# apple/swift-homomorphic-encryption

Measured on NVIDIA B200. Metric: BFV ct*ct mults/sec at N=8192, 4 coefficient moduli, higher is better.
Workload: dtype u64

## Files before the change

swift-homomorphic-encryption_b200/csrc/context.cu:

```cuda
#include "context.hpp"

#include <cuda_runtime.h>

#include <cmath>
#include <cstdlib>
#include <cstring>

#include "hostmath.hpp"
#include "ntt_fast.cuh"

namespace hecuda {
using namespace host;


static void fill_barrett(u64 p, u64 &mu1, u64 &mu_hi, u64 &mu_lo) {
    mu1 = (u64)(((u128)1 << 64) / p);
    u128 mu = (p & (p - 1)) == 0 ? ((u128)1 << (128 - (bit_length(p) - 1))) : (~(u128)0) / p;
    mu_hi = (u64)(mu >> 64);
    mu_lo = (u64)mu;
}

static bool build_slot(HostSlot &hs, u64 p, int64_t n, int logn, u64 t, std::vector<ulonglong2> &tw,
                       std::vector<ulonglong2> &itw, std::string &err) {
    if (!is_prime(p) || (p - 1) % (2 * (u64)n) != 0) {
        err = "invalidNttModulus: " + std::to_string(p) + " is not a prime = 1 mod 2N";
        return false;
    }
    if (p >= (1ull << 62)) {
        err = "invalidModulus: " + std::to_string(p) + " exceeds 2^62 - 1";
        return false;
    }
    ModSlot &d = hs.dev;
    std::memset(&d, 0, sizeof(d));
    d.p = p;
    fill_barrett(p, d.mu1, d.mu_hi, d.mu_lo);
    d.bits = bit_length(p);
    d.s_prod = d.bits - 2;
    d.mu_prod = (u64)(((u128)1 << (d.bits + 62)) / p);
    d.red_shift = d.bits > 12 ? d.bits - 12 : 0;
    d.red_recip = (u32)((((u128)1) << (d.red_shift + 32)) / p);
    const u64 psi = min_primitive_root(2 * (u64)n, p);
    const u64 psi_inv = invmod(psi, p);
    hs.roots.assign(n, 1);
    hs.inv_roots.assign(n, 1);
    u64 pw = 1, ipw = 1;
    for (int64_t i = 0; i < n; ++i) {
        unsigned r = bitrev((unsigned)i, logn);
        hs.roots[r] = pw;
        hs.inv_roots[r] = ipw;
        pw = mulmod(pw, psi, p);
        ipw = mulmod(ipw, psi_inv, p);
    }
    tw.resize(n);
    itw.resize(n);
    for (int64_t i = 0; i < n; ++i) {
        tw[i] = make_ulonglong2(hs.roots[i], shoup_factor(hs.roots[i], p));
        itw[i] = make_ulonglong2(hs.inv_roots[i], shoup_factor(hs.inv_roots[i], p));
    }
    const u64 n_inv = invmod((u64)n % p, p);
    const u64 w1_inv = n > 1 ? hs.inv_roots[1] : 1;
    d.r64 = (u64)(((u128)1 << 64) % p);
    {
        u64 inv = p;
        for (int i = 0; i < 6; ++i) inv *= 2 - p * inv;
        d.ninv = 0 - inv;
    }
    const u64 scalings[3] = {1 % p, mulmod(t % p, d.r64, p), d.r64};
    for (int k = 0; k < 3; ++k) {
        ModSlot::InvScale &sc = d.inv_scale[k];
        sc.c0 = mulmod(n_inv, scalings[k], p);
        sc.c0p = shoup_factor(sc.c0, p);
        sc.c1 = mulmod(sc.c0, w1_inv, p);
        sc.c1p = shoup_factor(sc.c1, p);
    }
    return true;
}

static DivRoundConsts build_divround(const std::vector<u64> &base) {
    DivRoundConsts c;
    std::memset(&c, 0, sizeof(c));
    c.l = (int)base.size();
    c.last = base.back();
    c.half = c.last >> 1;
    for (int i = 0; i + 1 < c.l; ++i) {
        const u64 m = base[i];
        c.m[i] = m;
        c.mu1[i] = (u64)(((u128)1 << 64) / m);
        c.half_mod[i] = c.half % m;
        c.inv_w[i] = invmod(c.last % m, m);
        c.inv_wp[i] = shoup_factor(c.inv_w[i], m);
    }
    return c;
}

Context *Context::create(int64_t n, const u64 *coeff_moduli, int nmod, u64 t, std::string &err, int word_bits) {
    if (word_bits != 64 && word_bits != 32) { err = "invalidEncryptionParameters: word size must be 32 or 64"; return nullptr; }
    for (int i = 0; i < nmod; ++i)
        if (coeff_moduli[i] >> (word_bits - 2)) { err = "invalidModulus: " + std::to_string(coeff_moduli[i]) + " exceeds the maximum of this word size"; return nullptr; }
    if (n < 2 || (n & (n - 1)) || n > (1 << 17)) { err = "invalidDegree: N must be a power of two in [2, 2^17]"; return nullptr; }
    if (n > (1 << fast::kSplitLogN)) { err = "unsupportedHeOperation: polynomial degrees above 2^" + std::to_string(fast::kSplitLogN) + " are not supported by the NTT kernels"; return nullptr; }
    if (nmod < 1) { err = "invalidEncryptionParameters: need at least one coefficient modulus"; return nullptr; }
    if (nmod > kMaxL) { err = "invalidEncryptionParameters: more than " + std::to_string(kMaxL) + " coefficient moduli (EncryptionParameters.swift:148)"; return nullptr; }
    if (t < 2) { err = "invalidEncryptionParameters: plaintext modulus"; return nullptr; }
    for (int i = 0; i < nmod; ++i)
        for (int j = 0; j < i; ++j)
            if (coeff_moduli[i] == coeff_moduli[j]) { err = "coprimeModuli: repeated coefficient modulus"; return nullptr; }

    Context *c = new Context();
    c->n = n;
    c->logn = bit_length((u64)n) - 1;
    c->has_ks = nmod >= 2;
    c->L = c->has_ks ? nmod - 1 : 1;
    c->t = t;
    c->word_bits = word_bits;
    c->mtilde = word_bits == 64 ? (1ull << 32) : (1ull << 16);
    c->gamma = word_bits == 64 ? ((1ull << 62) - 40797) : ((1ull << 30) - 20405);
    const u64 kMTilde = c->mtilde;
    cudaGetDevice(&c->device);
    c->sm_count = 1;
    cudaDeviceGetAttribute(&c->sm_count, cudaDevAttrMultiProcessorCount, c->device);
    const int L = c->L;
    c->q.assign(coeff_moduli, coeff_moduli + L);
    c->q_ks = c->has_ks ? coeff_moduli[L] : 0;
    for (u64 qi : c->q)
        if (t >= qi) { err = "invalidEncryptionParameters: plaintext modulus must be below every coefficient modulus"; delete c; return nullptr; }
    c->bsk = smallest_ntt_primes(word_bits - 3, L + 1, (u64)n);
    if ((int)c->bsk.size() != L + 1) { err = "notEnoughPrimes for Bsk"; delete c; return nullptr; }
    for (u64 b : c->bsk)
        for (int i = 0; i < nmod; ++i)
            if (b == coeff_moduli[i]) { err = "coprimeModuli: coefficient modulus collides with the BEHZ base"; delete c; return nullptr; }

    c->aux = c->bsk;
    {
        const char *env = std::getenv("HECUDA_AUX_BASE");
        const bool want_fast = !(env && std::string(env) == "reference");
        const int widths[2] = {30, 55};
        double log_q = 0;
        for (u64 v : c->q) log_q += std::log2((double)v);
        const double log_n = (double)c->logn, log_t = std::log2((double)t);
        for (int wi = 0; wi < 2 && want_fast && c->aux == c->bsk && word_bits == 64; ++wi) {
            const bool h_primes = fast::kNarrowHEnabled && std::getenv("HECUDA_AUX_H_PRIMES") != nullptr;
            std::vector<u64> cand = (widths[wi] == 55 && h_primes) ? smallest_ntt_primes(55, L + 1 + nmod, 1ull << 31)
                                                                   : smallest_ntt_primes(widths[wi], L + 1 + nmod, (u64)n);
            std::vector<u64> pick;
            for (u64 v : cand) {
                bool used = false;
                for (int i = 0; i < nmod; ++i) used |= coeff_moduli[i] == v;
                if (!used && (int)pick.size() < L + 1) pick.push_back(v);
            }
            double log_aux = 0, log_aux_l = 0;
            for (size_t j = 0; j < pick.size(); ++j) {
                log_aux += std::log2((double)pick[j]);
                if ((int)j < L) log_aux_l += std::log2((double)pick[j]);
            }
            const bool enough = (int)pick.size() == L + 1 && log_aux >= log_q + log_n + 4 &&
                                log_aux_l + std::log2((double)pick.back()) >= log_t + log_n + log_q + 5;
            if (enough) c->aux = pick;
        }
    }
    c->aux_is_reference = c->aux == c->bsk;

    const int nslots = c->aux_is_reference ? 2 * L + 2 : 3 * L + 3;
    c->slots.resize(nslots);
    std::vector<u64> slot_mod(nslots);
    for (int i = 0; i < L; ++i) slot_mod[c->slot_q(i)] = c->q[i];
    for (int j = 0; j <= L; ++j) slot_mod[c->slot_bsk(j)] = c->bsk[j];
    slot_mod[c->slot_ks()] = c->q_ks;
    if (!c->aux_is_reference)
        for (int j = 0; j <= L; ++j) slot_mod[c->slot_aux(j)] = c->aux[j];
    const size_t table_bytes = sizeof(ulonglong2) * (size_t)n;
    const bool fast = c->logn >= fast::kMinLogN && c->logn <= fast::kMaxLogN;
    const bool split = c->logn == fast::kSplitLogN;
    const int half_logn = c->logn - 1;
    const int64_t half_n = n / 2;
    const int threads = (int)((split ? half_n : n) / 16);
    const size_t tr_bytes = (fast || split) ? sizeof(ulonglong2) * (size_t)15 * threads : 0;
    const size_t half_bytes = sizeof(ulonglong2) * (size_t)half_n;
    const size_t slot_bytes = 2 * table_bytes + (split ? 2 * (2 * half_bytes + 2 * tr_bytes) : 2 * tr_bytes);
    if (cudaMalloc(&c->d_pool, slot_bytes * nslots) != cudaSuccess) { err = "cudaMalloc failed for twiddle tables"; delete c; return nullptr; }
    std::vector<ulonglong2> tw, itw, tr(15 * (size_t)threads), itr(15 * (size_t)threads), twh, itwh;
    std::vector<ModSlot> dev_slots(split ? 3 * nslots : nslots);
    c->split_slot_base = split ? nslots : 0;
    for (int s = 0; s < nslots; ++s) {
        if (s == c->slot_ks() && !c->has_ks) {
            std::memset(&c->slots[s].dev, 0, sizeof(ModSlot));
            dev_slots[s] = c->slots[s].dev;
            continue;
        }
        if (!build_slot(c->slots[s], slot_mod[s], n, c->logn, t, tw, itw, err)) { delete c; return nullptr; }
        char *base = (char *)c->d_pool + slot_bytes * s;
        cudaMemcpy(base, tw.data(), table_bytes, cudaMemcpyHostToDevice);
        cudaMemcpy(base + table_bytes, itw.data(), table_bytes, cudaMemcpyHostToDevice);
        c->slots[s].dev.tw = (const ulonglong2 *)base;
        c->slots[s].dev.itw = (const ulonglong2 *)(base + table_bytes);
        if (fast) {
            for (int k = 0; k < 15; ++k)
                for (int tau = 0; tau < threads; ++tau) {
                    tr[(size_t)k * threads + tau] = tw[fast::fwd_last_source(c->logn, k, tau)];
                    itr[(size_t)k * threads + tau] = itw[fast::inv_first_source(c->logn, k, tau)];
                }
            cudaMemcpy(base + 2 * table_bytes, tr.data(), tr_bytes, cudaMemcpyHostToDevice);
            cudaMemcpy(base + 2 * table_bytes + tr_bytes, itr.data(), tr_bytes, cudaMemcpyHostToDevice);
            c->slots[s].dev.tw_t = (const ulonglong2 *)(base + 2 * table_bytes);
            c->slots[s].dev.itw_t = (const ulonglong2 *)(base + 2 * table_bytes + tr_bytes);
        }
        dev_slots[s] = c->slots[s].dev;
        if (split) {
            for (int hh = 0; hh < 2; ++hh) {
                twh.assign(half_n, tw[0]);
                itwh.assign(half_n, itw[0]);
                for (int64_t i = 1; i < half_n; ++i) {
                    const int sp = bit_length((u64)i) - 1;
                    const int64_t src = ((int64_t)(2 + hh) << sp) + (i - ((int64_t)1 << sp));
                    twh[i] = tw[src];
                    itwh[i] = itw[src];
                }
                for (int k = 0; k < 15; ++k)
                    for (int tau = 0; tau < threads; ++tau) {
                        tr[(size_t)k * threads + tau] = twh[fast::fwd_last_source(half_logn, k, tau)];
                        itr[(size_t)k * threads + tau] = itwh[fast::inv_first_source(half_logn, k, tau)];
                    }
                char *hb = base + 2 * table_bytes + hh * (2 * half_bytes + 2 * tr_bytes);
// ... 203 lines not shown
```

swift-homomorphic-encryption_b200/csrc/context.hpp:

```cpp
#pragma once
#include <cstdint>
#include <string>
#include <vector>

#include "modarith.cuh"

namespace hecuda {

constexpr int kMaxL = 32;
constexpr int kMaxSlots = 3 * kMaxL + 3;
constexpr int kMaxRows = 2 * kMaxL + 1;

struct ModSlot {
    u64 p;
    u64 mu1;
    u64 mu_hi, mu_lo;
    u64 mu_prod;
    int s_prod;
    int bits;
    int red_shift;
    u32 red_recip;
    u64 ninv;
    u64 r64;
    struct InvScale { u64 c0, c0p, c1, c1p; } inv_scale[3];
    const ulonglong2 *tw;
    const ulonglong2 *itw;
    const ulonglong2 *tw_t;
    const ulonglong2 *itw_t;
};

enum { kScalePlain = 0, kScaleTMont = 1, kScaleMont = 2 };

struct NttRowMap {
    int rows_per_poly;
    int group;
    unsigned char slot[kMaxRows + 1];
    int src_mod;
    long long src_poly_stride;
    unsigned char src_slot[kMaxRows + 1];
};

struct LiftConsts {
    int L;
    int wide_sums;
    u64 b_mu1[kMaxL + 1];
    u64 q[kMaxL];
    u64 in_w[kMaxL], in_wp[kMaxL];
    u32 punct_mt[kMaxL];
    u32 neg_inv_q_mt;
    u32 mt_mask, mt_half;
    u64 neg_off[kMaxL + 1];
    u64 b[kMaxL + 1], b_ninv[kMaxL + 1];
    u64 mat[kMaxL + 1][kMaxL];
    u64 qr[kMaxL + 1];
};

// ... 75 lines not shown
```

swift-homomorphic-encryption_b200/csrc/hostmath.hpp:

```cpp
#pragma once
#include <cstdint>
#include <vector>

namespace hecuda {
namespace host {

typedef unsigned long long u64;
typedef unsigned __int128 u128;

inline u64 mulmod(u64 a, u64 b, u64 p) { return (u64)((u128)a * b % p); }

inline u64 powmod(u64 b, u64 e, u64 p) {
    u64 r = 1 % p;
    b %= p;
    for (; e; e >>= 1) {
        if (e & 1) r = mulmod(r, b, p);
        b = mulmod(b, b, p);
    }
    return r;
}

inline u64 invmod(u64 a, u64 m) {
    if (m == 0) return 0;
    a %= m;
// ... 11 lines not shown

inline bool is_prime(u64 n) {
    static const u64 witnesses[12] = {2, 3, 5, 7, 11, 13, 17, 19, 23, 29, 31, 37};
    if (n < 2) return false;
    for (u64 w : witnesses) {
        if (n == w) return true;
        if (n % w == 0) return false;
    }
    u64 d = n - 1;
    int r = 0;
    while (!(d & 1)) { d >>= 1; ++r; }
    for (u64 w : witnesses) {
        u64 x = powmod(w, d, n);
        if (x == 1 || x == n - 1) continue;
        bool composite = true;
        for (int i = 1; i < r && composite; ++i) {
            x = mulmod(x, x, n);
            if (x == n - 1) composite = false;
        }
        if (composite) return false;
    }
    return true;
}

inline std::vector<u64> smallest_ntt_primes(int bits, int count, u64 degree) {
    std::vector<u64> out;
    const u64 step = 2 * degree;
    const u64 lo = 1ull << (bits - 1), hi = (bits == 64) ? ~0ull : (1ull << bits);
    for (u64 c = lo + 1; c < hi && (int)out.size() < count; c += step)
        if (c % step == 1 && is_prime(c)) out.push_back(c);
    return out;
}

inline u64 min_primitive_root(u64 order, u64 p) {
    if (order < 2 || (order & (order - 1)) || (p - 1) % order) return 0;
    u64 gen = 0;
    for (u64 g = 2; g < p; ++g) {
        u64 r = powmod(g, (p - 1) / order, p);
        if (powmod(r, order / 2, p) == p - 1) { gen = r; break; }
    }
    if (!gen) return 0;
    u64 best = gen, cur = gen, g2 = mulmod(gen, gen, p);
    for (u64 k = 1; k < order; k += 2) {
        if (cur < best) best = cur;
        cur = mulmod(cur, g2, p);
    }
    return best;
}

inline unsigned bitrev(unsigned x, int bits) {
    unsigned r = 0;
    for (int i = 0; i < bits; ++i) r |= ((x >> i) & 1u) << (bits - 1 - i);
    return r;
}

inline int bit_length(u64 x) { return x ? 64 - __builtin_clzll(x) : 0; }

inline u64 prod_mod(const u64 *m, int n, u64 p) {
    u64 r = 1 % p;
    for (int i = 0; i < n; ++i) r = mulmod(r, m[i] % p, p);
    return r;
}
inline u64 punctured_mod(const u64 *m, int n, int skip, u64 p) {
    u64 r = 1 % p;
    for (int i = 0; i < n; ++i)
        if (i != skip) r = mulmod(r, m[i] % p, p);
// ... 7 lines not shown
```

swift-homomorphic-encryption_b200/csrc/ntt_fast.cu:

```cuda
#include <cuda.h>

#include <mutex>

#include <algorithm>
#include <cstdlib>
#include "kernels.cuh"
#include "ntt_fast.cuh"

namespace hecuda {
using namespace fast;

constexpr int kMaxRowList = 2 * (kMaxL + 1) * kMaxL;
struct RowList {
    int rows_per_poly;
    int count;
    unsigned short row[kMaxRowList];
    unsigned short slot[kMaxRowList];
    unsigned char flags[kMaxRowList];
    unsigned short src_row[kMaxRowList];
    long long src_poly_stride;
};

__device__ __forceinline__ u32 smem_u32(const void *p) { return (u32)__cvta_generic_to_shared(p); }
__device__ __forceinline__ void mbar_init(u64 *bar, int count) {
// ... 11 lines not shown
        "@!done bra WAIT_%=;\n\t}" ::"r"(smem_u32(bar)),
        "r"(parity)
        : "memory");
}
__device__ __forceinline__ void tma_load_1d(void *smem_dst, const void *gmem_src, u32 bytes, u64 *bar) {
    asm volatile("cp.async.bulk.shared::cluster.global.mbarrier::complete_tx::bytes [%0], [%1], %2, [%3];" ::"r"(smem_u32(smem_dst)),
                 "l"(gmem_src), "r"(bytes), "r"(smem_u32(bar))
                 : "memory");
}
__device__ __forceinline__ void tma_load_box(void *smem_dst, const CUtensorMap *map, int line, u64 *bar) {
    asm volatile("cp.async.bulk.tensor.2d.shared::cluster.global.tile.mbarrier::complete_tx::bytes [%0], [%1, {%2, %3}], [%4];" ::"r"(
                     smem_u32(smem_dst)),
                 "l"(map), "r"(0), "r"(line), "r"(smem_u32(bar))
                 : "memory");
}
__device__ __forceinline__ void tma_store_box(const CUtensorMap *map, int line, const void *smem_src) {
    asm volatile("cp.async.bulk.tensor.2d.global.shared::cta.tile.bulk_group [%0, {%1, %2}], [%3];" ::"l"(map), "r"(0), "r"(line),
                 "r"(smem_u32(smem_src))
                 : "memory");
}
__device__ __forceinline__ void tma_prefetch_box(const CUtensorMap *map, int line) {
    asm volatile("cp.async.bulk.prefetch.tensor.2d.L2.global.tile [%0, {%1, %2}];" ::"l"(map), "r"(0), "r"(line) : "memory");
}
__device__ __forceinline__ void tma_commit() { asm volatile("cp.async.bulk.commit_group;" ::: "memory"); }
__device__ __forceinline__ void tma_store_wait_read() { asm volatile("cp.async.bulk.wait_group.read 0;" ::: "memory"); }
__device__ __forceinline__ void tma_store_wait_all() { asm volatile("cp.async.bulk.wait_group 0;" ::: "memory"); }
__device__ __forceinline__ void fence_proxy_async_smem() { asm volatile("fence.proxy.async.shared::cta;" ::: "memory"); }

template <int LOGN, int CLS, int K>
__device__ __forceinline__ void fwd_row_pass(u64 (&x)[16], u64 *sm, int tau, const RowMod &m, bool reduce_in) {
    constexpr int P = plan_passes(LOGN), C = fwd_c(LOGN, K), LB = fwd_lb(LOGN, K);
    load_smem<LOGN, LB, C>(x, sm, tau);
    if (K == 0 && reduce_in) {
#pragma unroll
        for (int r = 0; r < 16; ++r) x[r] = barrett64(x[r], 0 - m.np, m.slot->mu1);
    }
    fwd_pass<LOGN, LB, C, CLS>(x, tau, m);
    if (K == P - 1) fwd_finish<CLS>(x, m);
    store_smem<LOGN, LB, C>(x, sm, tau);
}
template <int LOGN, int CLS>
__device__ __forceinline__ void fwd_row(u64 *sm, int tau, const RowMod &m, bool reduce_in) {
    constexpr int P = plan_passes(LOGN);
    u64 x[16];
    fwd_row_pass<LOGN, CLS, 0>(x, sm, tau, m, reduce_in);
    __syncthreads();
    fwd_row_pass<LOGN, CLS, 1>(x, sm, tau, m, false);
    __syncthreads();
    if (P == 4) {
        fwd_row_pass<LOGN, CLS, (P == 4 ? 2 : 1)>(x, sm, tau, m, false);
        __syncthreads();
    }
    fwd_row_pass<LOGN, CLS, P - 1>(x, sm, tau, m, false);
}

template <int LOGN, int CLS, int K>
__device__ __forceinline__ void inv_row_pass(u64 (&x)[16], u64 *sm, int tau, const RowMod &m) {
    constexpr int C = inv_c(LOGN, K), LB = inv_lb(LOGN, K);
    load_smem<LOGN, LB, C>(x, sm, tau);
    if (narrow_like(CLS) && K > 0 && inv_reduce_at(LOGN, K)) inv_reduce(x, m);
    inv_pass<LOGN, LB, C, CLS, inv_bound_in(LOGN, K)>(x, tau, m);
    if (K == plan_passes(LOGN) - 1 && m.partial) {
        if (CLS == kSmall) {
#pragma unroll
            for (int r = 0; r < 16; ++r) x[r] = csub32((u32)x[r], (u32)(0 - m.np));
        } else {
            reduce_small16(x, m);
        }
    }
    store_smem<LOGN, LB, C>(x, sm, tau);
}
template <int LOGN, int CLS>
__device__ __forceinline__ void inv_row(u64 *sm, int tau, const RowMod &m) {
    constexpr int P = plan_passes(LOGN);
    u64 x[16];
    inv_row_pass<LOGN, CLS, 0>(x, sm, tau, m);
    __syncthreads();
    inv_row_pass<LOGN, CLS, 1>(x, sm, tau, m);
    __syncthreads();
    if (P == 4) {
        inv_row_pass<LOGN, CLS, (P == 4 ? 2 : 1)>(x, sm, tau, m);
        __syncthreads();
    }
    inv_row_pass<LOGN, CLS, P - 1>(x, sm, tau, m);
}

template <int LOGN>
constexpr size_t ntt_smem_bytes() {
    return sizeof(u64) * ((size_t)1 << LOGN) + sizeof(ulonglong2) * ((size_t)1 << (LOGN - 4)) + 16;
}

template <int LOGN, bool INVERSE>
__global__ void __launch_bounds__((1 << LOGN) / 16, (1024 / ((1 << LOGN) / 16)))
    ntt_rows_kernel(const __grid_constant__ CUtensorMap map_in, const __grid_constant__ CUtensorMap map_out,
                    const ModSlot *__restrict__ slots, const __grid_constant__ RowList rl, const int polys,
                    const int scale_mode, const int debug_flags) {
    extern __shared__ __align__(1024) u64 sm[];
    constexpr int kLines = (1 << LOGN) / kLineWords;
    constexpr int kBoxes = kLines > kBoxLines ? kLines / kBoxLines : 1;
    constexpr int kLinesPerBox = kLines / kBoxes;
    constexpr u32 kRowBytes = (u32)sizeof(u64) << LOGN, kTwBytes = (u32)sizeof(ulonglong2) << (LOGN - 4);
    ulonglong2 *tw_cache = reinterpret_cast<ulonglong2 *>(sm + (1 << LOGN));
    u64 *bar_row = reinterpret_cast<u64 *>(tw_cache + (1 << (LOGN - 4)));
    u64 *bar_tw = bar_row + 1;
    const int tau = threadIdx.x;
    const int tasks = polys * rl.count;
    if (tau == 0) {
        if (smem_u32(sm) & 1023) __trap();
        mbar_init(bar_row, 1);
        mbar_init(bar_tw, 1);
    }
    __syncthreads();
    u32 phase_row = 0, phase_tw = 0;
    int cached_slot = -1;
    for (int task = blockIdx.x; task < tasks; task += gridDim.x) {
        const int which = task / polys;
        const int poly = task - which * polys;
        const int flags = rl.flags[which];
        const int slot = rl.slot[which];
        const ModSlot &S = slots[slot];
        const int64_t out_word = ((int64_t)poly * rl.rows_per_poly + rl.row[which]) << LOGN;
        const int64_t in_word = INVERSE ? out_word : (int64_t)poly * rl.src_poly_stride + ((int64_t)rl.src_row[which] << LOGN);
        const bool new_slot = slot != cached_slot;
        cached_slot = slot;
        if (tau == 0) {
            if (new_slot) {
                mbar_arrive_expect_tx(bar_tw, kTwBytes);
                tma_load_1d(tw_cache, INVERSE ? S.itw : S.tw, kTwBytes, bar_tw);
            }
            mbar_arrive_expect_tx(bar_row, kRowBytes);
            const int line = (int)(in_word >> 4);
#pragma unroll
            for (int b = 0; b < kBoxes; ++b) tma_load_box(sm + b * kLinesPerBox * kLineWords, &map_in, line + b * kLinesPerBox, bar_row);
            const int next = task + gridDim.x;
            if (next < tasks && !(debug_flags & 1)) {
                const int nw = next / polys;
                const int np_ = next - nw * polys;
                const int64_t nword = INVERSE ? ((int64_t)np_ * rl.rows_per_poly + rl.row[nw]) << LOGN
                                              : (int64_t)np_ * rl.src_poly_stride + ((int64_t)rl.src_row[nw] << LOGN);
#pragma unroll
                for (int b = 0; b < kBoxes; ++b) tma_prefetch_box(&map_in, (int)(nword >> 4) + b * kLinesPerBox);
            }
        }
        const int cls = flags & 7;
        RowMod m;
        m.np = 0 - S.p;
        m.kp = (cls == kWide || cls == kSmall) ? 2 * S.p : 4 * S.p;
        m.tw = nullptr;
        m.tw_s = smem_u32(tw_cache);
        m.slot = &S;
        m.scale_mode = INVERSE ? scale_mode : -1;
        m.partial = INVERSE && (flags & 16) != 0;
        if (new_slot) {
            mbar_wait(bar_tw, phase_tw);
            phase_tw ^= 1;
        }
        mbar_wait(bar_row, phase_row);
        phase_row ^= 1;
        if (debug_flags & 4) {
        } else
#ifndef HE_EXPERIMENT_ONLY_CLASS
        if (INVERSE) {
            if (kNarrowHEnabled && cls == kNarrowH) inv_row<LOGN, kNarrowHEnabled ? kNarrowH : kNarrow>(sm, tau, m);
            else if (cls == kNarrow) inv_row<LOGN, kNarrow>(sm, tau, m);
            else if (cls == kSmall) inv_row<LOGN, kSmall>(sm, tau, m);
            else if (cls == kMid) inv_row<LOGN, kMid>(sm, tau, m);
            else inv_row<LOGN, kWide>(sm, tau, m);
        } else {
            const bool reduce_in = (flags & 8) != 0;
            if (kNarrowHEnabled && cls == kNarrowH) fwd_row<LOGN, kNarrowHEnabled ? kNarrowH : kNarrow>(sm, tau, m, reduce_in);
            else if (cls == kNarrow) fwd_row<LOGN, kNarrow>(sm, tau, m, reduce_in);
            else if (cls == kSmall) fwd_row<LOGN, kSmall>(sm, tau, m, reduce_in);
            else if (cls == kMid) fwd_row<LOGN, kMid>(sm, tau, m, reduce_in);
            else fwd_row<LOGN, kWide>(sm, tau, m, reduce_in);
        }
#else
        if (INVERSE) inv_row<LOGN, HE_EXPERIMENT_ONLY_CLASS>(sm, tau, m);
        else fwd_row<LOGN, HE_EXPERIMENT_ONLY_CLASS>(sm, tau, m, (flags & 8) != 0);
#endif
        fence_proxy_async_smem();
        __syncthreads();
        if (tau == 0 && !(debug_flags & 2)) {
            const int line = (int)(out_word >> 4);
#pragma unroll
            for (int b = 0; b < kBoxes; ++b) tma_store_box(&map_out, line + b * kLinesPerBox, sm + b * kLinesPerBox * kLineWords);
            tma_commit();
            tma_store_wait_read();
        }
    }
    if (tau == 0) tma_store_wait_all();
}

static void build_row_list(const Context &ctx, const NttRowMap &map, bool inverse, RowList &rl) {
    rl.rows_per_poly = map.rows_per_poly;
    rl.count = 0;
    rl.src_poly_stride = map.src_mod ? map.src_poly_stride : (long long)map.rows_per_poly * ctx.n;
    static const int order[5] = {kWide, kMid, kNarrow, kNarrowH, kSmall};
    for (int oi = 0; oi < 5; ++oi) {
        const int cls = order[oi];
        for (int r = 0; r < map.rows_per_poly; ++r) {
            const int slot = map.slot[r / map.group];
            if (class_of_modulus(ctx.slots[slot].dev.p, ctx.slots[slot].dev.bits) != cls) continue;
            const int i = rl.count++;
            rl.row[i] = (unsigned short)r;
            rl.slot[i] = (unsigned short)slot;
            rl.src_row[i] = (unsigned short)(map.src_mod && !inverse ? r % map.src_mod : r);
            int flags = cls;
            if (map.src_mod && !inverse) {
                const u64 p = ctx.slots[slot].dev.p, src_p = ctx.slots[map.src_slot[r % map.src_mod]].dev.p;
                const u64 room = narrow_like(cls) ? 2u : cls == kMid ? 8u : cls == kSmall ? 1u : 4u;
                if (src_p > p && (src_p - 1) / p >= room) flags |= 8;
            }
            rl.flags[i] = (unsigned char)flags;
        }
    }
}

typedef CUresult (*EncodeTiledFn)(CUtensorMap *, CUtensorMapDataType, cuuint32_t, void *, const cuuint64_t *, const cuuint64_t *,
                                  const cuuint32_t *, const cuuint32_t *, CUtensorMapInterleave, CUtensorMapSwizzle,
                                  CUtensorMapL2promotion, CUtensorMapFloatOOBfill);
static EncodeTiledFn encode_tiled() {
    static EncodeTiledFn fn = [] {
        void *p = nullptr;
        cudaDriverEntryPointQueryResult q;
        if (cudaGetDriverEntryPoint("cuTensorMapEncodeTiled", &p, cudaEnableDefault, &q) != cudaSuccess || q != cudaDriverEntryPointSuccess)
            p = nullptr;
        return (EncodeTiledFn)p;
    }();
    return fn;
}
static bool make_line_map(CUtensorMap *map, const u64 *base, int logn) {
    EncodeTiledFn enc = encode_tiled();
    if (!enc || (reinterpret_cast<uintptr_t>(base) & 15)) return false;
    const int lines = (1 << logn) / kLineWords;
    const cuuint64_t dims[2] = {kLineWords, (cuuint64_t)1 << 31};
    const cuuint64_t strides[1] = {kLineWords * sizeof(u64)};
    const cuuint32_t box[2] = {kLineWords, (cuuint32_t)(lines > kBoxLines ? kBoxLines : lines)};
    const cuuint32_t elem_strides[2] = {1, 1};
    return enc(map, CU_TENSOR_MAP_DATA_TYPE_UINT64, 2, const_cast<u64 *>(base), dims, strides, box, elem_strides,
               CU_TENSOR_MAP_INTERLEAVE_NONE, CU_TENSOR_MAP_SWIZZLE_128B, CU_TENSOR_MAP_L2_PROMOTION_L2_128B,
               CU_TENSOR_MAP_FLOAT_OOB_FILL_NONE) == CUDA_SUCCESS;
}

template <int LOGN, bool INVERSE>
static cudaError_t launch_logn(const Context &ctx, const NttRowMap &map, const u64 *in, u64 *out, int64_t rows,
                               int scale_mode, cudaStream_t stream) {
    if (rows % map.rows_per_poly) return cudaErrorInvalidValue;
    if (rows == 0) return cudaSuccess;
    if (rows > 0x7fffffffLL) return cudaErrorInvalidValue;
    RowList rl;
    build_row_list(ctx, map, INVERSE, rl);
    if (rl.src_poly_stride % kLineWords) return cudaErrorInvalidValue;
    CUtensorMap map_in, map_out;
    if (!make_line_map(&map_in, in, LOGN) || !make_line_map(&map_out, out, LOGN)) return cudaErrorInvalidValue;
    const int polys = (int)(rows / map.rows_per_poly);
    constexpr int threads = (1 << LOGN) / 16;
    constexpr size_t smem = ntt_smem_bytes<LOGN>();
    auto k = ntt_rows_kernel<LOGN, INVERSE>;
    static int ctas_per_sm[64] = {0};
    static std::mutex mu;
    int per_sm;
    {
        std::lock_guard<std::mutex> lock(mu);
        int &c = ctas_per_sm[ctx.device & 63];
        if (c == 0) {
            cudaError_t e;
            if ((e = cudaFuncSetAttribute(k, cudaFuncAttributeMaxDynamicSharedMemorySize, (int)smem)) != cudaSuccess) return e;
            int n = 0;
            if ((e = cudaOccupancyMaxActiveBlocksPerMultiprocessor(&n, k, threads, smem)) != cudaSuccess) return e;
            if (n < 1) return cudaErrorInvalidConfiguration;
            c = n;
        }
        per_sm = c;
    }
    const int64_t grid = std::min<int64_t>(rows, (int64_t)ctx.sm_count * per_sm);
    ++g_kernel_launches;
    static const int debug_flags = [] {
        const char *env = std::getenv("HECUDA_NTT_DEBUG");
        return env ? std::atoi(env) : 0;
    }();
    k<<<(unsigned)grid, threads, smem, stream>>>(map_in, map_out, ctx.d_slots, rl, polys, scale_mode, debug_flags);
    return cudaGetLastError();
}

struct SplitRows {
    int rows_per_poly, count;
    unsigned short row[kMaxRowList];
    unsigned short src_row[kMaxRowList], slot[kMaxRowList];
    unsigned char reduce_in[kMaxRowList];
    long long src_poly_stride;
};
__global__ void __launch_bounds__(256) ntt_split_forward_kernel(const u64 *__restrict__ in, u64 *__restrict__ out,
                                                               const ModSlot *__restrict__ slots,
                                                               const __grid_constant__ SplitRows sr, int polys, int logn) {
    const int64_t n = (int64_t)1 << logn, half = n >> 1;
    const int which = blockIdx.y;
    const int64_t poly = blockIdx.z;
// ... 46 lines not shown
    sr.rows_per_poly = full.rows_per_poly;
    sr.count = full.count;
    sr.src_poly_stride = full.src_poly_stride;
    RowList rl;
    rl.rows_per_poly = 2 * full.rows_per_poly;
    rl.count = 2 * full.count;
    rl.src_poly_stride = (long long)rl.rows_per_poly << LOGN;
    for (int i = 0; i < full.count; ++i) {
        sr.row[i] = full.row[i];
        sr.slot[i] = full.slot[i];
        sr.src_row[i] = full.src_row[i];
        sr.reduce_in[i] = (unsigned char)((map.src_mod && !INVERSE) ? 1 : 0);
        for (int hh = 0; hh < 2; ++hh) {
            const int j = 2 * i + hh;
            rl.row[j] = (unsigned short)(2 * full.row[i] + hh);
            rl.src_row[j] = rl.row[j];
            rl.slot[j] = (unsigned short)(ctx.split_slot_base + 2 * full.slot[i] + hh);
            rl.flags[j] = (unsigned char)((full.flags[i] & 7) | (INVERSE ? 16 : 0));
        }
    }
    const dim3 egrid((unsigned)((ctx.n / 4 + 255) / 256), (unsigned)full.count, (unsigned)polys);
    if (!INVERSE) {
        ++g_kernel_launches;
        ntt_split_forward_kernel<<<egrid, 256, 0, stream>>>(in, out, ctx.d_slots, sr, polys, ctx.logn);
        cudaError_t e = cudaGetLastError();
        if (e != cudaSuccess) return e;
        in = out;
    }
    CUtensorMap map_in, map_out;
    if (!make_line_map(&map_in, in, LOGN) || !make_line_map(&map_out, out, LOGN)) return cudaErrorInvalidValue;
    {
        constexpr int threads = (1 << LOGN) / 16;
        constexpr size_t smem = ntt_smem_bytes<LOGN>();
        auto k = ntt_rows_kernel<LOGN, INVERSE>;
        cudaError_t e;
        if ((e = cudaFuncSetAttribute(k, cudaFuncAttributeMaxDynamicSharedMemorySize, (int)smem)) != cudaSuccess) return e;
        int per_sm = 0;
        if ((e = cudaOccupancyMaxActiveBlocksPerMultiprocessor(&per_sm, k, threads, smem)) != cudaSuccess) return e;
        if (per_sm < 1) return cudaErrorInvalidConfiguration;
        const int64_t grid = std::min<int64_t>(2 * rows, (int64_t)ctx.sm_count * per_sm);
        ++g_kernel_launches;
        k<<<(unsigned)grid, threads, smem, stream>>>(map_in, map_out, ctx.d_slots, rl, polys, scale_mode, 0);
        if ((e = cudaGetLastError()) != cudaSuccess) return e;
    }
    if (INVERSE) {
        ++g_kernel_launches;
        ntt_merge_inverse_kernel<<<egrid, 256, 0, stream>>>(out, ctx.d_slots, sr, polys, ctx.logn, scale_mode);
        return cudaGetLastError();
    }
    return cudaSuccess;
}

bool ntt_fast_supported(const Context &ctx) { return ctx.logn >= kMinLogN && ctx.logn <= kSplitLogN; }

template <bool INVERSE>
static cudaError_t launch_fast(const Context &ctx, const NttRowMap &map, const u64 *in, u64 *out, int64_t rows,
                               int scale_mode, cudaStream_t stream) {
    switch (ctx.logn) {
        case 10: return launch_logn<10, INVERSE>(ctx, map, in, out, rows, scale_mode, stream);
        case 11: return launch_logn<11, INVERSE>(ctx, map, in, out, rows, scale_mode, stream);
        case 12: return launch_logn<12, INVERSE>(ctx, map, in, out, rows, scale_mode, stream);
        case 13: return launch_logn<13, INVERSE>(ctx, map, in, out, rows, scale_mode, stream);
        case 14: return launch_logn<14, INVERSE>(ctx, map, in, out, rows, scale_mode, stream);
        case 15: return launch_split<INVERSE>(ctx, map, in, out, rows, scale_mode, stream);
        default: return cudaErrorInvalidValue;
    }
}
// ... 12 lines not shown
```

swift-homomorphic-encryption_b200/csrc/ntt_fast.cuh:

```cuda
#pragma once
#include "context.hpp"
#include "modarith.cuh"

namespace hecuda {
namespace fast {

constexpr int kMinLogN = 10, kMaxLogN = 14;
constexpr int kSplitLogN = 15;
constexpr int kNarrowBits = 55;
constexpr int kMidBits = 61;
constexpr int kSmallBits = 30;
enum { kNarrow = 0, kMid = 1, kWide = 2, kSmall = 3, kNarrowH = 4 };
HE_HD constexpr int class_of_bits(int bits) {
    return bits <= kSmallBits ? kSmall : bits <= kNarrowBits ? kNarrow : bits <= kMidBits ? kMid : kWide;
}
#if defined(HE_NTT_NARROW_H)
constexpr bool kNarrowHEnabled = true;
#else
constexpr bool kNarrowHEnabled = false;
#endif
HE_HD constexpr int class_of_modulus(u64 p, int bits) {
    return (kNarrowHEnabled && class_of_bits(bits) == kNarrow && (u32)p == 1u) ? kNarrowH : class_of_bits(bits);
}
HE_HD constexpr bool narrow_like(int cls) { return cls == kNarrow || cls == kNarrowH; }

HE_HD constexpr int plan_passes(int logn) { return logn <= 12 ? 3 : 4; }
HE_HD constexpr int plan_c(int logn, int k) {
    return logn == 10   ? (k == 2 ? 4 : 3)
           : logn == 11 ? (k == 1 ? 3 : 4)
           : logn == 12 ? 4
           : logn == 13 ? (k == 3 ? 4 : 3)
                        : (k == 0 || k == 3 ? 4 : 3);
}
HE_HD constexpr int fwd_c(int logn, int k) { return plan_c(logn, k); }
HE_HD constexpr int fwd_lb(int logn, int k) {
    int s0 = 0;
    for (int i = 0; i < k; ++i) s0 += plan_c(logn, i);
    return logn - s0 - plan_c(logn, k);
}
HE_HD constexpr int inv_c(int logn, int k) { return plan_c(logn, plan_passes(logn) - 1 - k); }
HE_HD constexpr int inv_lb(int logn, int k) {
    int u0 = 0;
    for (int i = 0; i < k; ++i) u0 += inv_c(logn, i);
    return u0;
}
// ... 234 lines not shown
    const u64 h = (0 - np) >> 32;
    return y * w - q - ((u64)((u32)q * (u32)h) << 32);
#endif
}
template <int CLS>
HE_HD u64 shoup4c(u64 y, u64 w, u64 wp, u64 np) { return CLS == kNarrowH ? shoup4h(y, w, wp, np) : shoup4(y, w, wp, np); }
HE_HD u64 shoup2(u64 y, u64 w, u64 wp, u64 np) { return y * w + mulhi64(y, wp) * np; }

HE_HD u64 reduce_small(u64 x, const u64 p, const u64 np, const int red_shift, const u32 red_recip) {
    const u32 xs = (u32)(x >> red_shift);
    const u32 qhat = mul_hi_u32(xs, red_recip);
    u32 np0, np1, rl, rh;
    unpack64(np, np0, np1);
    unpack64(mad_wide_u32(qhat, np0, x), rl, rh);
    rh = qhat * np1 + rh;
    return csub(pack64(rl, rh), p);
}
HE_HD void reduce_small16(u64 (&x)[16], const RowMod &m) {
    const int shift = m.slot->red_shift;
    const u32 recip = m.slot->red_recip;
    const u64 p = 0 - m.np;
#pragma unroll
    for (int r = 0; r < 16; ++r) x[r] = reduce_small(x[r], p, m.np, shift, recip);
}

HE_HD u32 csub32(u32 x, u32 m) {
    const u32 d = x - m;
    return d < x ? d : x;
}
HE_HD u32 shoup32(u32 y, u32 w, u32 wp, u32 p) {
    return y * w - mul_hi_u32(y, wp) * p;
}

template <int CLS>
HE_HD void ct_butterfly(u64 &x, u64 &y, const ulonglong2 w, const RowMod &m) {
    if (CLS == kSmall) {
        const u32 p = (u32)(0 - m.np), p2 = 2 * p;
        const u32 xr = csub32((u32)x, p2);
        const u32 v = shoup32((u32)y, (u32)w.x, (u32)(w.y >> 32), p);
        x = xr + v;
        y = xr - v + p2;
    } else if (narrow_like(CLS)) {
        const u64 v = shoup4c<CLS>(y, w.x, w.y, m.np);
        const u64 xo = x + v;
        y = x - v + m.kp;
        x = xo;
    } else if (CLS == kMid) {
        const u64 xr = csub(x, m.kp);
        const u64 v = shoup4(y, w.x, w.y, m.np);
        x = xr + v;
        y = xr - v + m.kp;
    } else {
        const u64 xr = csub(x, m.kp);
        const u64 v = shoup2(y, w.x, w.y, m.np);
        x = xr + v;
        y = xr - v + m.kp;
    }
}

template <int LOGN, int LB, int C, int CLS>
HE_HD void fwd_pass(u64 (&x)[16], int tau, const RowMod &m) {
    constexpr int E = pass_e(LB, C), F = 1 << E, S0 = LOGN - LB - C, T = (1 << LOGN) / 16;
    const int hi = tau >> (LB - E);
    const ulonglong2 *tw_t = LB == 0 ? m.tw_t() + tau : nullptr;
#pragma unroll
    for (int j = 0; j < C; ++j) {
        const int h = 1 << (C - 1 - j);
#pragma unroll
        for (int grp = 0; grp < (1 << j); ++grp) {
            const ulonglong2 w = LB == 0 ? ld_tw(tw_t + ((1 << j) - 1 + grp) * T)
                                         : ld_tw_cached(m, (1 << (S0 + j)) + (hi << j) + grp);
#pragma unroll
            for (int k = 0; k < h; ++k) {
                const int a = grp * 2 * h + k;
#pragma unroll
                for (int f = 0; f < F; ++f) ct_butterfly<CLS>(x[a * F + f], x[(a + h) * F + f], w, m);
            }
        }
    }
}

template <int CLS>
HE_HD void fwd_finish(u64 (&x)[16], const RowMod &m) {
    if (CLS == kSmall) {
        const u32 p = (u32)(0 - m.np);
#pragma unroll
        for (int r = 0; r < 16; ++r) x[r] = csub32(csub32((u32)x[r], 2 * p), p);
    } else {
        reduce_small16(x, m);
    }
}

template <int CLS>
HE_HD void gs_butterfly(u64 &x, u64 &y, const ulonglong2 w, const RowMod &m, u64 kp) {
    if (CLS == kSmall) {
        const u32 p = (u32)(0 - m.np), p2 = 2 * p;
        const u32 s = csub32((u32)x + (u32)y, p2);
        y = shoup32((u32)x - (u32)y + p2, (u32)w.x, (u32)(w.y >> 32), p);
        x = s;
    } else if (narrow_like(CLS)) {
        const u64 s = x + y;
        y = shoup4c<CLS>(x - y + kp, w.x, w.y, m.np);
        x = s;
    } else if (CLS == kMid) {
        const u64 s = csub(x + y, kp);
        y = shoup4(x - y + kp, w.x, w.y, m.np);
        x = s;
    } else {
        const u64 s = csub(x + y, kp);
        y = shoup2(x - y + kp, w.x, w.y, m.np);
        x = s;
    }
}

template <int LOGN, int LB, int C, int CLS, int BIN, int J>
HE_HD void inv_stage(u64 (&x)[16], const int tau, const RowMod &m) {
    constexpr int E = pass_e(LB, C), F = 1 << E, T = (1 << LOGN) / 16;
    constexpr int HH = 1 << J;
    constexpr bool kLast = (LB + J == LOGN - 1);
    constexpr int kGroups = 1 << (LOGN - 1 - LB - J);
    const int hi = tau >> (LB - E);
    const u64 kp = narrow_like(CLS) ? (0 - m.np) * (u64)inv_bound_after(BIN, J) : m.kp;
    const ulonglong2 *tw_t = LB == 0 ? m.tw_t() + tau : nullptr;
#pragma unroll
    for (int grp = 0; grp < (1 << (C - 1 - J)); ++grp) {
        if (!kLast || m.partial) {
            const ulonglong2 w = LB == 0 ? ld_tw(tw_t + (16 - (16 >> J) + grp) * T)
                                         : ld_tw_cached(m, kGroups + (hi << (C - 1 - J)) + grp);
#pragma unroll
            for (int k = 0; k < HH; ++k) {
                const int a = grp * 2 * HH + k;
#pragma unroll
                for (int f = 0; f < F; ++f) gs_butterfly<CLS>(x[a * F + f], x[(a + HH) * F + f], w, m, kp);
            }
        } else {
            const u64 *sc = &m.slot->inv_scale[m.scale_mode].c0;
            const u64 c0 = ld_u64(sc), c0p = ld_u64(sc + 1), c1 = ld_u64(sc + 2), c1p = ld_u64(sc + 3);
#pragma unroll
            for (int k = 0; k < HH; ++k) {
                const int a = grp * 2 * HH + k;
#pragma unroll
                for (int f = 0; f < F; ++f) {
                    if (CLS == kSmall) {
                        const u32 p = (u32)(0 - m.np);
                        const u32 xa = (u32)x[a * F + f], ya = (u32)x[(a + HH) * F + f];
                        x[a * F + f] = csub32(shoup32(xa + ya, (u32)c0, (u32)(c0p >> 32), p), p);
                        x[(a + HH) * F + f] = csub32(shoup32(xa - ya + 2 * p, (u32)c1, (u32)(c1p >> 32), p), p);
                        continue;
                    }
                    const u64 xa = x[a * F + f], ya = x[(a + HH) * F + f];
                    const u64 s = xa + ya;
                    const u64 d = xa - ya + kp;
                    x[a * F + f] = csub(shoup2(s, c0, c0p, m.np), 0 - m.np);
                    x[(a + HH) * F + f] = csub(shoup2(d, c1, c1p, m.np), 0 - m.np);
                }
            }
        }
    }
}

template <int LOGN, int LB, int C, int CLS, int BIN>
HE_HD void inv_pass(u64 (&x)[16], int tau, const RowMod &m) {
    inv_stage<LOGN, LB, C, CLS, BIN, 0>(x, tau, m);
    if (C > 1) inv_stage<LOGN, LB, C, CLS, BIN, (C > 1 ? 1 : 0)>(x, tau, m);
    if (C > 2) inv_stage<LOGN, LB, C, CLS, BIN, (C > 2 ? 2 : 0)>(x, tau, m);
    if (C > 3) inv_stage<LOGN, LB, C, CLS, BIN, (C > 3 ? 3 : 0)>(x, tau, m);
}

HE_HD void inv_reduce(u64 (&x)[16], const RowMod &m) { reduce_small16(x, m); }

HE_HD int fwd_last_source(int logn, int k, int tau) {
    int j = 0;
    while ((2 << j) - 1 <= k) ++j;
    const int grp = k - ((1 << j) - 1);
    return (1 << (logn - 4 + j)) + (tau << j) + grp;
// ... 11 lines not shown
```

Before: 186,000.

## Add FP64-based NTT path for 51-bit auxiliary BEHZ primes

Result: faster. 204,600, median of 6 (+10.0%).

```diff
diff --git a/swift-homomorphic-encryption_b200/csrc/context.cu b/swift-homomorphic-encryption_b200/csrc/context.cu
--- a/swift-homomorphic-encryption_b200/csrc/context.cu
+++ b/swift-homomorphic-encryption_b200/csrc/context.cu
@@ -20,8 +20,13 @@
     mu_lo = (u64)mu;
 }
 
+static ulonglong2 f64_constant(u64 w, u64 p) {
+    const double wc = w > p / 2 ? -(double)(p - w) : (double)w;
+    return make_ulonglong2(fast::f64_bits(wc), fast::f64_bits(wc / (double)p));
+}
+
 static bool build_slot(HostSlot &hs, u64 p, int64_t n, int logn, u64 t, std::vector<ulonglong2> &tw,
-                       std::vector<ulonglong2> &itw, std::string &err) {
+                       std::vector<ulonglong2> &itw, std::string &err, bool f64 = false) {
     if (!is_prime(p) || (p - 1) % (2 * (u64)n) != 0) {
         err = "invalidNttModulus: " + std::to_string(p) + " is not a prime = 1 mod 2N";
         return false;
@@ -54,9 +59,11 @@
     tw.resize(n);
     itw.resize(n);
     for (int64_t i = 0; i < n; ++i) {
-        tw[i] = make_ulonglong2(hs.roots[i], shoup_factor(hs.roots[i], p));
-        itw[i] = make_ulonglong2(hs.inv_roots[i], shoup_factor(hs.inv_roots[i], p));
-    }
+        tw[i] = f64 ? f64_constant(hs.roots[i], p) : make_ulonglong2(hs.roots[i], shoup_factor(hs.roots[i], p));
+        itw[i] = f64 ? f64_constant(hs.inv_roots[i], p) : make_ulonglong2(hs.inv_roots[i], shoup_factor(hs.inv_roots[i], p));
+    }
+    d.f64 = f64 ? 1 : 0;
+    d.pinv = 1.0 / (double)p;
     const u64 n_inv = invmod((u64)n % p, p);
     const u64 w1_inv = n > 1 ? hs.inv_roots[1] : 1;
     d.r64 = (u64)(((u128)1 << 64) % p);
@@ -72,6 +79,10 @@
         sc.c0p = shoup_factor(sc.c0, p);
         sc.c1 = mulmod(sc.c0, w1_inv, p);
         sc.c1p = shoup_factor(sc.c1, p);
+        if (f64) {
+            const ulonglong2 a = f64_constant(sc.c0, p), b = f64_constant(sc.c1, p);
+            sc = {a.x, a.y, b.x, b.y};
+        }
     }
     return true;
 }
@@ -131,17 +142,24 @@
             if (b == coeff_moduli[i]) { err = "coprimeModuli: coefficient modulus collides with the BEHZ base"; delete c; return nullptr; }
 
     c->aux = c->bsk;
+    const bool fast = c->logn >= fast::kMinLogN && c->logn <= fast::kMaxLogN;
+    bool aux_f64 = false;
     {
         const char *env = std::getenv("HECUDA_AUX_BASE");
         const bool want_fast = !(env && std::string(env) == "reference");
-        const int widths[2] = {30, 55};
+        const bool want_51 = !(env && std::string(env) == "narrow") && fast;
+        const char *env_f64 = std::getenv("HECUDA_NTT_F64"), *env_impl = std::getenv("HECUDA_NTT_IMPL");
+        const bool want_f64 = !(env_f64 && std::string(env_f64) == "0") && !(env_impl && std::string(env_impl) == "simple");
+        const int widths[3] = {30, 51, 55};
         double log_q = 0;
         for (u64 v : c->q) log_q += std::log2((double)v);
         const double log_n = (double)c->logn, log_t = std::log2((double)t);
-        for (int wi = 0; wi < 2 && want_fast && c->aux == c->bsk && word_bits == 64; ++wi) {
+        for (int wi = 0; wi < 3 && want_fast && c->aux == c->bsk && word_bits == 64; ++wi) {
+            if (widths[wi] == 51 && !want_51) continue;
             const bool h_primes = fast::kNarrowHEnabled && std::getenv("HECUDA_AUX_H_PRIMES") != nullptr;
             std::vector<u64> cand = (widths[wi] == 55 && h_primes) ? smallest_ntt_primes(55, L + 1 + nmod, 1ull << 31)
-                                                                   : smallest_ntt_primes(widths[wi], L + 1 + nmod, (u64)n);
+                                    : widths[wi] == 51               ? largest_ntt_primes(51, L + 1 + nmod, (u64)n)
+                                                                     : smallest_ntt_primes(widths[wi], L + 1 + nmod, (u64)n);
             std::vector<u64> pick;
             for (u64 v : cand) {
                 bool used = false;
@@ -155,7 +173,10 @@
             }
             const bool enough = (int)pick.size() == L + 1 && log_aux >= log_q + log_n + 4 &&
                                 log_aux_l + std::log2((double)pick.back()) >= log_t + log_n + log_q + 5;
-            if (enough) c->aux = pick;
+            if (enough) {
+                c->aux = pick;
+                aux_f64 = widths[wi] == 51 && want_f64;
+            }
         }
     }
     c->aux_is_reference = c->aux == c->bsk;
@@ -169,7 +190,6 @@
     if (!c->aux_is_reference)
         for (int j = 0; j <= L; ++j) slot_mod[c->slot_aux(j)] = c->aux[j];
     const size_t table_bytes = sizeof(ulonglong2) * (size_t)n;
-    const bool fast = c->logn >= fast::kMinLogN && c->logn <= fast::kMaxLogN;
     const bool split = c->logn == fast::kSplitLogN;
     const int half_logn = c->logn - 1;
     const int64_t half_n = n / 2;
@@ -187,7 +207,8 @@
             dev_slots[s] = c->slots[s].dev;
             continue;
         }
-        if (!build_slot(c->slots[s], slot_mod[s], n, c->logn, t, tw, itw, err)) { delete c; return nullptr; }
+        const bool f64 = aux_f64 && s >= c->slot_aux(0);
+        if (!build_slot(c->slots[s], slot_mod[s], n, c->logn, t, tw, itw, err, f64)) { delete c; return nullptr; }
         char *base = (char *)c->d_pool + slot_bytes * s;
         cudaMemcpy(base, tw.data(), table_bytes, cudaMemcpyHostToDevice);
         cudaMemcpy(base + table_bytes, itw.data(), table_bytes, cudaMemcpyHostToDevice);
diff --git a/swift-homomorphic-encryption_b200/csrc/context.hpp b/swift-homomorphic-encryption_b200/csrc/context.hpp
--- a/swift-homomorphic-encryption_b200/csrc/context.hpp
+++ b/swift-homomorphic-encryption_b200/csrc/context.hpp
@@ -22,6 +22,8 @@
     u32 red_recip;
     u64 ninv;
     u64 r64;
+    int f64;
+    double pinv;
     struct InvScale { u64 c0, c0p, c1, c1p; } inv_scale[3];
     const ulonglong2 *tw;
     const ulonglong2 *itw;
diff --git a/swift-homomorphic-encryption_b200/csrc/hostmath.hpp b/swift-homomorphic-encryption_b200/csrc/hostmath.hpp
--- a/swift-homomorphic-encryption_b200/csrc/hostmath.hpp
+++ b/swift-homomorphic-encryption_b200/csrc/hostmath.hpp
@@ -67,6 +67,14 @@
     return out;
 }
 
+inline std::vector<u64> largest_ntt_primes(int bits, int count, u64 degree) {
+    std::vector<u64> out;
+    const u64 step = 2 * degree, lo = 1ull << (bits - 1);
+    for (u64 c = ((1ull << bits) - 1) / step * step + 1; c > lo && (int)out.size() < count; c -= step)
+        if (is_prime(c)) out.push_back(c);
+    return out;
+}
+
 inline u64 min_primitive_root(u64 order, u64 p) {
     if (order < 2 || (order & (order - 1)) || (p - 1) % order) return 0;
     u64 gen = 0;
diff --git a/swift-homomorphic-encryption_b200/csrc/ntt_fast.cu b/swift-homomorphic-encryption_b200/csrc/ntt_fast.cu
--- a/swift-homomorphic-encryption_b200/csrc/ntt_fast.cu
+++ b/swift-homomorphic-encryption_b200/csrc/ntt_fast.cu
@@ -67,9 +67,11 @@
     constexpr int P = plan_passes(LOGN), C = fwd_c(LOGN, K), LB = fwd_lb(LOGN, K);
     load_smem<LOGN, LB, C>(x, sm, tau);
     if (K == 0 && reduce_in) {
+        const u64 p = CLS == kF64 ? m.slot->p : 0 - m.np;
 #pragma unroll
-        for (int r = 0; r < 16; ++r) x[r] = barrett64(x[r], 0 - m.np, m.slot->mu1);
-    }
+        for (int r = 0; r < 16; ++r) x[r] = barrett64(x[r], p, m.slot->mu1);
+    }
+    if (K == 0) to_f64_16<CLS>(x);
     fwd_pass<LOGN, LB, C, CLS>(x, tau, m);
     if (K == P - 1) fwd_finish<CLS>(x, m);
     store_smem<LOGN, LB, C>(x, sm, tau);
@@ -93,9 +95,10 @@
 __device__ __forceinline__ void inv_row_pass(u64 (&x)[16], u64 *sm, int tau, const RowMod &m) {
     constexpr int C = inv_c(LOGN, K), LB = inv_lb(LOGN, K);
     load_smem<LOGN, LB, C>(x, sm, tau);
+    if (K == 0) to_f64_16<CLS>(x);
     if (narrow_like(CLS) && K > 0 && inv_reduce_at(LOGN, K)) inv_reduce(x, m);
     inv_pass<LOGN, LB, C, CLS, inv_bound_in(LOGN, K)>(x, tau, m);
-    if (K == plan_passes(LOGN) - 1 && m.partial) {
+    if (CLS != kF64 && K == plan_passes(LOGN) - 1 && m.partial) {
         if (CLS == kSmall) {
 #pragma unroll
             for (int r = 0; r < 16; ++r) x[r] = csub32((u32)x[r], (u32)(0 - m.np));
@@ -125,7 +128,7 @@
     return sizeof(u64) * ((size_t)1 << LOGN) + sizeof(ulonglong2) * ((size_t)1 << (LOGN - 4)) + 16;
 }
 
-template <int LOGN, bool INVERSE>
+template <int LOGN, bool INVERSE, bool F64>
 __global__ void __launch_bounds__((1 << LOGN) / 16, (1024 / ((1 << LOGN) / 16)))
     ntt_rows_kernel(const __grid_constant__ CUtensorMap map_in, const __grid_constant__ CUtensorMap map_out,
                     const ModSlot *__restrict__ slots, const __grid_constant__ RowList rl, const int polys,
@@ -179,8 +182,8 @@
         }
         const int cls = flags & 7;
         RowMod m;
-        m.np = 0 - S.p;
-        m.kp = (cls == kWide || cls == kSmall) ? 2 * S.p : 4 * S.p;
+        m.np = F64 && cls == kF64 ? f64_bits(S.pinv) : 0 - S.p;
+        m.kp = F64 && cls == kF64 ? f64_bits(u64_to_f64(S.p)) : (cls == kWide || cls == kSmall) ? 2 * S.p : 4 * S.p;
         m.tw = nullptr;
         m.tw_s = smem_u32(tw_cache);
         m.slot = &S;
@@ -196,14 +199,16 @@
         } else
 #ifndef HE_EXPERIMENT_ONLY_CLASS
         if (INVERSE) {
-            if (kNarrowHEnabled && cls == kNarrowH) inv_row<LOGN, kNarrowHEnabled ? kNarrowH : kNarrow>(sm, tau, m);
+            if (F64 && cls == kF64) inv_row<LOGN, kF64>(sm, tau, m);
+            else if (kNarrowHEnabled && cls == kNarrowH) inv_row<LOGN, kNarrowHEnabled ? kNarrowH : kNarrow>(sm, tau, m);
             else if (cls == kNarrow) inv_row<LOGN, kNarrow>(sm, tau, m);
             else if (cls == kSmall) inv_row<LOGN, kSmall>(sm, tau, m);
             else if (cls == kMid) inv_row<LOGN, kMid>(sm, tau, m);
             else inv_row<LOGN, kWide>(sm, tau, m);
         } else {
             const bool reduce_in = (flags & 8) != 0;
-            if (kNarrowHEnabled && cls == kNarrowH) fwd_row<LOGN, kNarrowHEnabled ? kNarrowH : kNarrow>(sm, tau, m, reduce_in);
+            if (F64 && cls == kF64) fwd_row<LOGN, kF64>(sm, tau, m, reduce_in);
+            else if (kNarrowHEnabled && cls == kNarrowH) fwd_row<LOGN, kNarrowHEnabled ? kNarrowH : kNarrow>(sm, tau, m, reduce_in);
             else if (cls == kNarrow) fwd_row<LOGN, kNarrow>(sm, tau, m, reduce_in);
             else if (cls == kSmall) fwd_row<LOGN, kSmall>(sm, tau, m, reduce_in);
             else if (cls == kMid) fwd_row<LOGN, kMid>(sm, tau, m, reduce_in);
@@ -230,12 +235,13 @@
     rl.rows_per_poly = map.rows_per_poly;
     rl.count = 0;
     rl.src_poly_stride = map.src_mod ? map.src_poly_stride : (long long)map.rows_per_poly * ctx.n;
-    static const int order[5] = {kWide, kMid, kNarrow, kNarrowH, kSmall};
-    for (int oi = 0; oi < 5; ++oi) {
+    static const int order[6] = {kWide, kMid, kNarrow, kNarrowH, kF64, kSmall};
+    for (int oi = 0; oi < 6; ++oi) {
         const int cls = order[oi];
         for (int r = 0; r < map.rows_per_poly; ++r) {
             const int slot = map.slot[r / map.group];
-            if (class_of_modulus(ctx.slots[slot].dev.p, ctx.slots[slot].dev.bits) != cls) continue;
+            const ModSlot &S = ctx.slots[slot].dev;
+            if ((S.f64 ? kF64 : class_of_modulus(S.p, S.bits)) != cls) continue;
             const int i = rl.count++;
             rl.row[i] = (unsigned short)r;
             rl.slot[i] = (unsigned short)slot;
@@ -243,7 +249,7 @@
             int flags = cls;
             if (map.src_mod && !inverse) {
                 const u64 p = ctx.slots[slot].dev.p, src_p = ctx.slots[map.src_slot[r % map.src_mod]].dev.p;
-                const u64 room = narrow_like(cls) ? 2u : cls == kMid ? 8u : cls == kSmall ? 1u : 4u;
+                const u64 room = narrow_like(cls) ? 2u : cls == kMid ? 8u : (cls == kSmall || cls == kF64) ? 1u : 4u;
                 if (src_p > p && (src_p - 1) / p >= room) flags |= 8;
             }
             rl.flags[i] = (unsigned char)flags;
@@ -291,13 +297,15 @@
     const int polys = (int)(rows / map.rows_per_poly);
     constexpr int threads = (1 << LOGN) / 16;
     constexpr size_t smem = ntt_smem_bytes<LOGN>();
-    auto k = ntt_rows_kernel<LOGN, INVERSE>;
-    static int ctas_per_sm[64] = {0};
+    bool f64 = false;
+    for (int i = 0; i < rl.count; ++i) f64 |= (rl.flags[i] & 7) == kF64;
+    auto k = f64 ? ntt_rows_kernel<LOGN, INVERSE, true> : ntt_rows_kernel<LOGN, INVERSE, false>;
+    static int ctas_per_sm[2][64] = {{0}};
     static std::mutex mu;
     int per_sm;
     {
         std::lock_guard<std::mutex> lock(mu);
-        int &c = ctas_per_sm[ctx.device & 63];
+        int &c = ctas_per_sm[f64][ctx.device & 63];
         if (c == 0) {
             cudaError_t e;
             if ((e = cudaFuncSetAttribute(k, cudaFuncAttributeMaxDynamicSharedMemorySize, (int)smem)) != cudaSuccess) return e;
@@ -410,7 +418,7 @@
     {
         constexpr int threads = (1 << LOGN) / 16;
         constexpr size_t smem = ntt_smem_bytes<LOGN>();
-        auto k = ntt_rows_kernel<LOGN, INVERSE>;
+        auto k = ntt_rows_kernel<LOGN, INVERSE, false>;
         cudaError_t e;
         if ((e = cudaFuncSetAttribute(k, cudaFuncAttributeMaxDynamicSharedMemorySize, (int)smem)) != cudaSuccess) return e;
         int per_sm = 0;
diff --git a/swift-homomorphic-encryption_b200/csrc/ntt_fast.cuh b/swift-homomorphic-encryption_b200/csrc/ntt_fast.cuh
--- a/swift-homomorphic-encryption_b200/csrc/ntt_fast.cuh
+++ b/swift-homomorphic-encryption_b200/csrc/ntt_fast.cuh
@@ -1,4 +1,7 @@
 #pragma once
+#include <cmath>
+#include <cstring>
+
 #include "context.hpp"
 #include "modarith.cuh"
 
@@ -10,7 +13,8 @@
 constexpr int kNarrowBits = 55;
 constexpr int kMidBits = 61;
 constexpr int kSmallBits = 30;
-enum { kNarrow = 0, kMid = 1, kWide = 2, kSmall = 3, kNarrowH = 4 };
+constexpr int kF64Bits = 51;
+enum { kNarrow = 0, kMid = 1, kWide = 2, kSmall = 3, kNarrowH = 4, kF64 = 5 };
 HE_HD constexpr int class_of_bits(int bits) {
     return bits <= kSmallBits ? kSmall : bits <= kNarrowBits ? kNarrow : bits <= kMidBits ? kMid : kWide;
 }
@@ -311,9 +315,84 @@
     return y * w - mul_hi_u32(y, wp) * p;
 }
 
+constexpr double kRoundMagic = 6755399441055744.0;
+constexpr double kTwo52 = 4503599627370496.0;
+HE_HD double as_f64(u64 v) {
+#if defined(__CUDA_ARCH__)
+    return __longlong_as_double((long long)v);
+#else
+    double d;
+    std::memcpy(&d, &v, sizeof d);
+    return d;
+#endif
+}
+HE_HD u64 f64_bits(double d) {
+#if defined(__CUDA_ARCH__)
+    return (u64)__double_as_longlong(d);
+#else
+    u64 v;
+    std::memcpy(&v, &d, sizeof v);
+    return v;
+#endif
+}
+HE_HD double f64_add(double a, double b) {
+#if defined(__CUDA_ARCH__)
+    return __dadd_rn(a, b);
+#else
+    return a + b;
+#endif
+}
+HE_HD double f64_mul(double a, double b) {
+#if defined(__CUDA_ARCH__)
+    return __dmul_rn(a, b);
+#else
+    return a * b;
+#endif
+}
+HE_HD double f64_fma(double a, double b, double c) {
+#if defined(__CUDA_ARCH__)
+    return __fma_rn(a, b, c);
+#else
+    return std::fma(a, b, c);
+#endif
+}
+HE_HD double f64_round_mul(double a, double b) { return f64_add(f64_fma(a, b, kRoundMagic), -kRoundMagic); }
+HE_HD double mulmod_f64(double y, double w, double wp, double p) {
+    const double h = f64_mul(y, w);
+    const double l = f64_fma(y, w, -h);
+    return f64_add(f64_fma(-f64_round_mul(y, wp), p, h), l);
+}
+HE_HD double reduce_f64(double x, double pinv, double p) { return f64_fma(-f64_round_mul(x, pinv), p, x); }
+HE_HD double u64_to_f64(u64 x) { return f64_add(as_f64(x | 0x4330000000000000ull), -kTwo52); }
+HE_HD u64 f64_to_canonical(double r, u64 p) {
+    const u64 v = (f64_bits(f64_add(r, kRoundMagic)) & ((1ull << 52) - 1)) - (1ull << 51);
+    return (long long)v < 0 ? v + p : v;
+}
+HE_HD constexpr bool f64_fwd_reduce_at(int s) {
+    int b = 8;
+    bool red = false;
+    for (int i = 0; i <= s; ++i) {
+        red = b > 16;
+        if (red) b = 5;
+        b += 5;
+    }
+    return red;
+}
+template <int CLS>
+HE_HD void to_f64_16(u64 (&x)[16]) {
+    if (CLS == kF64) {
+#pragma unroll
+        for (int r = 0; r < 16; ++r) x[r] = f64_bits(u64_to_f64(x[r]));
+    }
+}
+
 template <int CLS>
 HE_HD void ct_butterfly(u64 &x, u64 &y, const ulonglong2 w, const RowMod &m) {
-    if (CLS == kSmall) {
+    if (CLS == kF64) {
+        const double v = mulmod_f64(as_f64(y), as_f64(w.x), as_f64(w.y), as_f64(m.kp)), xd = as_f64(x);
+        x = f64_bits(f64_add(xd, v));
+        y = f64_bits(f64_add(xd, -v));
+    } else if (CLS == kSmall) {
         const u32 p = (u32)(0 - m.np), p2 = 2 * p;
         const u32 xr = csub32((u32)x, p2);
         const u32 v = shoup32((u32)y, (u32)w.x, (u32)(w.y >> 32), p);
@@ -344,6 +423,11 @@
     const ulonglong2 *tw_t = LB == 0 ? m.tw_t() + tau : nullptr;
 #pragma unroll
     for (int j = 0; j < C; ++j) {
+        if (CLS == kF64 && f64_fwd_reduce_at(S0 + j)) {
+            const double p = as_f64(m.kp), pinv = as_f64(m.np);
+#pragma unroll
+            for (int r = 0; r < 16; ++r) x[r] = f64_bits(reduce_f64(as_f64(x[r]), pinv, p));
+        }
         const int h = 1 << (C - 1 - j);
 #pragma unroll
         for (int grp = 0; grp < (1 << j); ++grp) {
@@ -361,7 +445,12 @@
 
 template <int CLS>
 HE_HD void fwd_finish(u64 (&x)[16], const RowMod &m) {
-    if (CLS == kSmall) {
+    if (CLS == kF64) {
+        const double p = as_f64(m.kp), pinv = as_f64(m.np);
+        const u64 pi = m.slot->p;
+#pragma unroll
+        for (int r = 0; r < 16; ++r) x[r] = f64_to_canonical(reduce_f64(as_f64(x[r]), pinv, p), pi);
+    } else if (CLS == kSmall) {
         const u32 p = (u32)(0 - m.np);
 #pragma unroll
         for (int r = 0; r < 16; ++r) x[r] = csub32(csub32((u32)x[r], 2 * p), p);
@@ -372,7 +461,11 @@
 
 template <int CLS>
 HE_HD void gs_butterfly(u64 &x, u64 &y, const ulonglong2 w, const RowMod &m, u64 kp) {
-    if (CLS == kSmall) {
+    if (CLS == kF64) {
+        const double p = as_f64(m.kp), xd = as_f64(x), yd = as_f64(y);
+        y = f64_bits(mulmod_f64(f64_add(xd, -yd), as_f64(w.x), as_f64(w.y), p));
+        x = f64_bits(reduce_f64(f64_add(xd, yd), as_f64(m.np), p));
+    } else if (CLS == kSmall) {
         const u32 p = (u32)(0 - m.np), p2 = 2 * p;
         const u32 s = csub32((u32)x + (u32)y, p2);
         y = shoup32((u32)x - (u32)y + p2, (u32)w.x, (u32)(w.y >> 32), p);
@@ -420,6 +513,13 @@
                 const int a = grp * 2 * HH + k;
 #pragma unroll
                 for (int f = 0; f < F; ++f) {
+                    if (CLS == kF64) {
+                        const double p = as_f64(m.kp), xa = as_f64(x[a * F + f]), ya = as_f64(x[(a + HH) * F + f]);
+                        const u64 pi = m.slot->p;
+                        x[a * F + f] = f64_to_canonical(mulmod_f64(f64_add(xa, ya), as_f64(c0), as_f64(c0p), p), pi);
+                        x[(a + HH) * F + f] = f64_to_canonical(mulmod_f64(f64_add(xa, -ya), as_f64(c1), as_f64(c1p), p), pi);
+                        continue;
+                    }
                     if (CLS == kSmall) {
                         const u32 p = (u32)(0 - m.np);
                         const u32 xa = (u32)x[a * F + f], ya = (u32)x[(a + HH) * F + f];
```
